# leducthanhig/image-restoration-models

Hardware: AMD Instinct MI355X
Metric: images/sec + PSNR, Restormer motion-deblur 1280x720 (higher is better)
Workload: dtype f32 (1x1 convs: fp32 emulated by 3 fp16 MFMAs on hi/lo operand splits with fp32 accumulation, error vs float64 at the level of an fp32 chain; everything else exact f32; value_exact_f32: f32 MFMA everywhere); 1 GPU; Restormer motion-deblur (WithBias LN, 26.13M params, synthetic weights seed 42) on 1280x720x3 uint8 GoPro-shaped synthetic frames; 6 tiles 512x512 (overlap 96) per frame; a step = 4 frame(s) per GPU, their 24 tiles in one batched forward; global_batch=4, tile=512, overlap=96, parallelism=per-image shard x1, no data-path collective

## Files before the change

image-restoration-models_amd/_hip.py:

```python
from __future__ import annotations

import ctypes as C
import os

import torch

_HERE = os.path.dirname(os.path.abspath(__file__))
LIB_PATH = os.path.join(_HERE, "libirm_hip.so")

ACT_NONE, ACT_RELU, ACT_GELU, ACT_SILU, ACT_RELU6 = 0, 1, 2, 3, 4
LN_NONE, LN_WITHBIAS, LN_BIASFREE = 0, 1, 2

_P, _L, _I, _F, _D = C.c_void_p, C.c_long, C.c_int, C.c_float, C.c_double

SIGNATURES = {
    "irm_version": [],
    "irm_ln_stats_f32": [_P, _L, _P, _I, _I, _I, _F, _P],
    "irm_gemm1x1_f32": [_P, _L, _P, _L, _P, _L, _P, _L, _P, _P, _P, _P, _I, _I, _I, _I, _I, _I, _I, _I, _P, _F, _P, _P],
    "irm_gemm1x1_f16x3_f32": [_P, _L, _P, _L, _P, _L, _P, _L, _P, _P, _P, _P, _I, _I, _I, _I, _I, _I, _I, _I, _P, _F, _P, _P],
    "irm_ln_split_f16": [_P, _L, _P, _P, _I, _F, _F, _P, _I, _I, _I, _P],
    "irm_ln_gemm_presplit_f16x3_f32": [_P, _P, _L, _P, _P, _I, _F, _F, _P, _L, _P, _F, _I, _I, _I, _I, _I, _P],
    "irm_ln_gemm_presplit_cl_f16x3_f32": [_P, _P, _L, _P, _P, _I, _F, _F, _P, _L, _P, _F, _I, _I, _I, _I, _I, _I, _P],
    "irm_gdfn_tail_f16x3_f32": [_P, _L, _P, _P, _P, _P, _L, _F, _I, _I, _I, _I, _I, _I, _P],
    "irm_gemm_presplit_f16x3_f32": [_P, _P, _P, _L, _P, _F, _I, _I, _I, _I, _I, _I, _I, _I, _P],
    "irm_dwconv3x3_f32": [_P, _L, _P, _P, _P, _L, _I, _I, _I, _I, _I, _P],
    "irm_dwconv3x3_gate_f32": [_P, _L, _P, _P, _P, _L, _I, _I, _I, _I, _P],
    "irm_dwgemm_f32": [_P, _L, _P, _P, _L, _P, _L, _P, _L, _P, _I, _I, _I, _I, _I, _I, _P, _F, _P],
    "irm_dwgemm_f16x3_f32": [_P, _L, _P, _P, _L, _P, _L, _P, _L, _P, _I, _I, _I, _I, _I, _I, _P, _F, _P],
    "irm_gdfn_fused_f16x3_f32": [_P, _P, _P, _P, _L, _P, _L, _I, _F, _F, _F, _I, _I, _I, _I, _I, _P],
    "irm_qkv_dw_fused_f16x3_f32": [_P, _P, _L, _P, _L, _I, _F, _F, _I, _I, _I, _I, _I, _P],
    "irm_mdta_gram_f32": [_P, _L, _P, _I, _I, _I, _I, _I, _P],
    "irm_mdta_gram_f16x3_f32": [_P, _L, _P, _P, _I, _I, _I, _I, _I, _P],
    "irm_mdta_finalize_f32": [_P, _P, _P, _P, _P, _P, _I, _I, _I, _I, _P],
    "irm_mdta_finalize_f16x3_f32": [_P, _P, _P, _P, _P, _P, _I, _I, _I, _I, _P],
    "irm_qkv_dw_fused_tm_f16x3_f32": [_P, _P, _L, _P, _L, _I, _F, _F, _I, _I, _I, _I, _I, _I, _P],
    "irm_qkv_gram_cm_f16x3_f32": [_P, _P, _L, _P, _L, _P, _P, _I, _F, _F, _I, _I, _I, _I, _I, _I, _P],
    "irm_qkv_dw_cm_f16x3_f32": [_P, _P, _L, _P, _L, _I, _F, _F, _I, _I, _I, _I, _I, _I, _P],
    "irm_mdta_gram_tm_f16x3_f32": [_P, _L, _P, _P, _I, _I, _I, _I, _I, _P],
    "irm_mdta_gram_tm_f32": [_P, _L, _P, _I, _I, _I, _I, _I, _P],
    "irm_mdta_finalize_frag_f16x3_f32": [_P, _P, _P, _P, _P, _P, _I, _I, _I, _I, _P],
    "irm_attn_gdfn_fused_f16x3_f32": [_P, _P, _P, _P, _L, _P, _L, _P, _P, _P, _L, _I, _F, _F, _F, _I, _I, _I, _I, _I, _I, _P],
    "irm_conv3x3_f32": [_P, _P, _L, _P, _L, _P, _L, _P, _I, _I, _I, _I, _I, _I, _I, _I, _I, _I, _I, _P],
    "irm_conv3x3_thin_f32": [_P, _P, _L, _P, _L, _P, _L, _P, _I, _I, _I, _I, _I, _I, _I, _I, _P],
    "irm_conv3x3_f16x3_f32": [_P, _F, _P, _L, _P, _L, _P, _L, _P, _I, _I, _I, _I, _I, _I, _I, _I, _I, _I, _I, _P],
    "irm_conv3x3_ep_f32": [_P, _P, _L, _P, _L, _P, _L, _P, _I, _I, _I, _I, _I, _I, _F, _I, _I, _I, _I, _I, _I, _P],
    "irm_conv3x3_f16x3_ep_f32": [_P, _F, _P, _L, _P, _L, _P, _L, _P, _I, _I, _I, _I, _I, _I, _F, _I, _I, _I, _I, _I, _I, _P],
    "irm_tile_extract": [_P, _I, _P, _P, _P, _I, _I, _I, _I, _I, _I, _I, _I, _F, _F, _I, _P],
    "irm_chan_stats_f32": [_P, _L, _P, _I, _I, _I, _F, _P],
    "irm_chan_stats_ws_f32": [_P, _L, _P, _P, _L, _I, _I, _I, _F, _P],
    "irm_chan_norm_act_f32": [_P, _L, _P, _P, _P, _P, _L, _P, _L, _I, _I, _I, _I, _P],
    "irm_conv3x3_s2_f32": [_P, _L, _P, _P, _L, _I, _I, _I, _I, _I, _P],
    "irm_dwconv3x3_s2_f32": [_P, _L, _P, _P, _L, _I, _I, _I, _I, _P],
    "irm_upsample_add_f32": [_P, _L, _P, _L, _P, _L, _I, _I, _I, _I, _I, _P],
    "irm_transpose_f32": [_P, _L, _P, _L, _I, _I, _I, _P],
    "irm_selective_scan_f32": [_P, _P, _P, _P, _P, _P, _P, _P, _P, _P, _P, _I, _I, _I, _I, _I, _I, _P],
    "irm_losh_combine_f32": [_P, _P, _P, _P, _P, _P, _P, _P, _L, _P, _L, _I, _I, _I, _I, _F, _P],
    "irm_window_blend": [_P, _P, _P, _P, _I, _P, _P, _I, _I, _I, _I, _I, _I, _I, _I, _I, _I, _F, _F, _P],
    "irm_window_blend_scaled": [_P, _P, _P, _P, _I, _P, _P, _I, _I, _I, _I, _I, _I, _I, _I, _I, _I, _I, _F, _F, _P],
    "irm_frame_metrics": [_P, _P, _I, _I, _I, _I, _I, _D, _P, _P, _P, _L, _P],
    "irm_imresize_bicubic": [_P, _I, _P, _I, _P, _P, _P, _P, _I, _I, _I, _I, _I, _I, _P],
    "irm_frame_metrics_basicsr": [_P, _P, _I, _I, _I, _I, _I, _I, _I, _I, _P, _P, _P, _L, _P],
    "irm_dihedral_chop_f32": [_P, _P, _P, _L, _I, _I, _I, _I, _I, _I, _I, _P],
    "irm_ensemble_merge_f32": [_P, _P, _P, _L, _I, _I, _I, _I, _I, _I, _P],
}

_lib = None


class HipLibraryError(RuntimeError):
    pass


def load():
    global _lib, LIB_PATH
    if _lib is None:
        if os.environ.get("IRM_HIP_LIB"):
            LIB_PATH = os.path.abspath(os.environ["IRM_HIP_LIB"])
        if not os.path.exists(LIB_PATH):
            raise HipLibraryError(
                f"{LIB_PATH} not found: build it with `python -c 'import __graft_entry__ as g; g.build()'` "
                "(make -C image-restoration-models_amd/csrc).  There is no CPU fallback.")
        lib = C.CDLL(LIB_PATH)
        for name, argtypes in SIGNATURES.items():
            fn = getattr(lib, name)
            fn.argtypes = argtypes
            fn.restype = _I
        _lib = lib
    return _lib


def _stream() -> int:
    return torch.cuda.current_stream().cuda_stream


def ptr(t):
    if t is None:
        return None
    if isinstance(t, int):
        return t
    assert t.is_cuda, "HIP kernels need device tensors"
    return t.data_ptr()


def call(name: str, *args):
    rc = getattr(load(), name)(*args, _stream())
    if rc != 0:
        raise HipLibraryError(f"{name} failed with status {rc} "
                              f"({'invalid arguments' if rc == -1 else 'HIP launch error'})")



def pack_gemm_weight(w: torch.Tensor) -> torch.Tensor:
    w = w.detach().reshape(w.shape[0], -1).float()
    m, k = w.shape
    mt, ks = (m + 15) // 16, 4 * ((k + 15) // 16)
    wpad = torch.zeros(mt * 16, ks * 4, dtype=torch.float32, device=w.device)
    wpad[:m, :k] = w
    return wpad.view(mt, 16, ks, 4).permute(0, 2, 3, 1).contiguous().view(-1)

# ... 381 lines not shown
```

image-restoration-models_amd/ops.py:

```python
from __future__ import annotations

import os

import torch

from . import _hip
from ._hip import ACT_GELU, ACT_NONE, ACT_RELU, ACT_RELU6, ACT_SILU, LN_BIASFREE, LN_NONE, LN_WITHBIAS


class KernelTimer:

    def __init__(self, detail=False, only=None):
        self.records = []
        self.detail = detail
        self.only = None if only is None else frozenset(only)
        self._chain = {}
        self._done = {}
        self._since = 0

    def _fold(self, k, e0, e1, fl, by):
        d = self._done.setdefault(k, dict(launches=0, ms=0.0, flops=0.0, bytes=0.0))
        d["launches"] += 1
        d["ms"] += e0.elapsed_time(e1)
        d["flops"] += fl
# ... 245 lines not shown
    ks = (C + 31) // 32
    return 2 * ks * ks * 512


def attn_gdfn_fused(pk, x, v, mfold_frag, y, C: int, hid: int, *, ln_mode, bias_o=None, bias=None, eps: float = 1e-5,
                    x_tm: bool = False, v_tm: bool = False, y_tm: bool = False):
    _chk(x, "x"), _chk(y, "y"), _chk(v, "v")
    B, _, H, W = x.shape
    assert x.data_ptr() != y.data_ptr() and x.shape[1] >= C and y.shape[1] >= C and v.shape[1] >= C and C % 16 == 0
    assert v.shape[0] == B and v.shape[2:] == x.shape[2:] and mfold_frag.numel() >= B * mfold_frag_numel(C)
    rec, w2, inv_s1, inv_s2 = pk
    N = H * W
    flops = B * N * (2.0 * C * C + 2.0 * 2 * hid * C + 36.0 * hid + 2.0 * hid * C)
    _launch("attn_gdfn_fused", flops, 4.0 * B * N * 3 * C, "irm_attn_gdfn_fused_f16x3_f32", _hip.ptr(rec), _hip.ptr(w2),
            _hip.ptr(bias), _hip.ptr(x), _bs(x), _hip.ptr(v), _bs(v), _hip.ptr(mfold_frag), _hip.ptr(bias_o),
            _hip.ptr(y), _bs(y), int(ln_mode), float(eps), float(inv_s1), float(inv_s2), B, C, hid, H, W,
            int(x_tm) | 2 * int(v_tm) | 4 * int(y_tm), tag=f"C{C} hid{hid} {H}x{W} B{B}")


def can_qk_tile_major(C: int, heads: int, H: int, W: int) -> bool:
    return C % 16 == 0 and C % heads == 0 and C // heads in (48, 96) and H % 8 == 0 and W % 32 == 0


def _use_qkv_cm(C: int) -> bool:
    return C <= 64


def qkv_dw_fused(pk, x, y, C: int, M: int, *, ln_mode, eps: float = 1e-5, tm: bool = False, x_tm: bool = False,
                 v_tm: bool = False):
    _chk(x, "x"), _chk(y, "y")
    B, _, H, W = x.shape
    assert x.data_ptr() != y.data_ptr() and x.shape[1] >= C and y.shape[1] >= M
    rec, inv_s1 = pk
    N = H * W
    if tm:
        assert M == 3 * C and y.shape[1] == M and H % 8 == 0 and W % 32 == 0
        _launch("qkv_dw_fused", B * N * (2.0 * M * C + 18.0 * M), 4.0 * B * N * (C + M),
                "irm_qkv_dw_cm_f16x3_f32" if _use_qkv_cm(C) else "irm_qkv_dw_fused_tm_f16x3_f32",
                _hip.ptr(rec), _hip.ptr(x), _bs(x), _hip.ptr(y), _bs(y), int(ln_mode), float(eps), float(inv_s1), B, C,
                H, W, int(x_tm), int(v_tm), tag=f"C{C} M{M} {H}x{W} B{B} tm")
        return
    assert not (x_tm or v_tm), "tile-major x / v need tm=True"
    _launch("qkv_dw_fused", B * N * (2.0 * M * C + 18.0 * M), 4.0 * B * N * (C + M), "irm_qkv_dw_fused_f16x3_f32",
            _hip.ptr(rec), _hip.ptr(x), _bs(x), _hip.ptr(y), _bs(y), int(ln_mode), float(eps), float(inv_s1), B, C, M,
            H, W, tag=f"C{C} M{M} {H}x{W} B{B}")


def mdta_plan(B: int, C: int, heads: int, N: int):
    c = C // heads
    sb = 3 if c % 48 == 0 else 2 if c % 32 == 0 else 1
    rec = c * c + 2 * c
    if c in (48, 96) and N % 64 == 0:
        slots, best = 2 * 256, None
        for chunk in range(128, 4096 + 1, 64):
            nchunk = -(-N // chunk)
            cost = -(-(B * heads * nchunk) // slots) * (chunk + 192)
            if best is None or cost < best[0]:
                best = (cost, chunk, nchunk)
        return best[1], best[2], rec
    nsub = (c // (16 * sb)) ** 2
    chunk = -(-(N * B * heads * nsub) // (4 * target_blocks()))
    chunk = min(max(-(-chunk // 64) * 64, 256), 4096)
    return chunk, -(-N // chunk), rec


QKV_GRAM_NCH = 4


def can_qkv_gram(C: int, heads: int, H: int, W: int) -> bool:
    return C == 48 and heads == 1 and H % 8 == 0 and W % 32 == 0 and ((H // 8) * (W // 32)) % QKV_GRAM_NCH == 0


def qkv_gram_cm(pk, x, y, gram_scale, part, C: int, *, ln_mode, eps: float = 1e-5, x_tm: bool = False, v_tm: bool = False) -> int:
    _chk(x, "x"), _chk(y, "y")
    B, _, H, W = x.shape
    assert can_qkv_gram(C, 1, H, W) and y.shape[1] == 3 * C and gram_scale.numel() == 2 * C
    rec, inv_s1 = pk
    N = H * W
    nchunk = (H // 8) * (W // 32) // QKV_GRAM_NCH
    assert part.numel() >= B * nchunk * (C * C + 2 * C)
    _launch("qkv_dw_fused", B * N * (2.0 * 3 * C * C + 18.0 * 3 * C + 2.0 * C * C), 4.0 * B * N * 2 * C, "irm_qkv_gram_cm_f16x3_f32",
            _hip.ptr(rec), _hip.ptr(x), _bs(x), _hip.ptr(y), _bs(y), _hip.ptr(gram_scale), _hip.ptr(part), int(ln_mode),
            float(eps), float(inv_s1), B, C, H, W, int(x_tm), int(v_tm), tag=f"C{C} {H}x{W} B{B} gram")
    return nchunk


def mdta_fold(qkv, part, gsum, temperature, wout, mfold, C: int, heads: int, attn=None, split: bool = False,
              gram_scale=None, frag: bool = False, tm: bool = False, nchunk_ready: int | None = None):
    _chk(qkv, "qkv")
    B, _, H, W = qkv.shape
    N = H * W
    chunk, nchunk, rec = mdta_plan(B, C, heads, N)
    if nchunk_ready is not None:
        nchunk = nchunk_ready
    assert part.numel() >= B * heads * nchunk * rec and gsum.numel() >= B * heads * rec
    c = C // heads
    assert not tm or (c in (48, 96) and N % 256 == 0), "tile-major q, k: the LDS-DMA ring passes only"
    if nchunk_ready is not None:
        pass
    elif gram_scale is not None and c in (48, 96) and N % 64 == 0:
        assert gram_scale.numel() == 2 * C and gram_scale.is_contiguous()
        _launch("mdta_gram_f16x3", 2.0 * B * heads * c * c * N, 8.0 * B * C * N,
                "irm_mdta_gram_tm_f16x3_f32" if tm else "irm_mdta_gram_f16x3_f32", _hip.ptr(qkv),
                _bs(qkv), _hip.ptr(gram_scale), _hip.ptr(part), B, C, heads, N, chunk,
                tag=f"C{C} h{heads} N{N} B{B} chunk{chunk}")
    else:
        _launch("mdta_gram", 2.0 * B * heads * c * c * N, 8.0 * B * C * N, "irm_mdta_gram_tm_f32" if tm else "irm_mdta_gram_f32",
                _hip.ptr(qkv), _bs(qkv), _hip.ptr(part), B, C, heads, N, chunk, tag=f"C{C} h{heads} N{N} B{B} chunk{chunk}")
    _launch("mdta_finalize", 2.0 * B * C * C * c, 4.0 * B * (heads * nchunk * rec + C * C),
            "irm_mdta_finalize_frag_f16x3_f32" if frag else "irm_mdta_finalize_f16x3_f32" if split else "irm_mdta_finalize_f32",
            _hip.ptr(part), _hip.ptr(gsum), _hip.ptr(temperature), _hip.ptr(wout), _hip.ptr(mfold), _hip.ptr(attn),
            B, C, heads, nchunk, tag=f"C{C} h{heads} nchunk{nchunk} B{B}")


def can_fuse_stats(M: int) -> bool:
    mt = (M + 15) // 16
    return mt <= _hip.choose_ct(mt)


def mfold_numel(C: int) -> int:
    mt = (C + 15) // 16
    return mt * 4 * mt * 64


def plan_conv3x3(co: int, H: int, W: int, B: int, *, split: bool, ct: int | None = None, ygroups: int | None = None):
    mt = (co + 15) // 16
    blocks = -(-W // 32) * -(-H // 8) * B
    if split:
        if ct is None:
            ct = 12 if mt >= 12 else 8 if mt >= 8 else 4 if mt % 4 == 0 else 3 if mt % 3 == 0 or mt > 4 else min(mt, 4)
            while ct > 1 and blocks * -(-mt // ct) < 256:
                ct = {12: 8, 8: 4}.get(ct, ct - 1)
        if ygroups is None:
            nchunks = -(-mt // ct)
            ygroups = max(1, min(nchunks, -(-512 // blocks)))
            while nchunks % ygroups:
                ygroups += 1
        return ct, ygroups
    if ct is None:
        ct = _hip.choose_ct(mt, (6, 4, 3, 2, 1))
        for smaller in (4, 3, 2, 1):
            if blocks * -(-mt // ct) >= 256 or smaller >= ct:
                continue
            ct = smaller
    if ygroups is None:
        nchunks = -(-mt // ct)
        ygroups = max(1, min(nchunks, -(-target_blocks() // blocks)))
    return ct, ygroups


def conv3x3(wp, x, y, ci: int, co: int, *, bias=None, relu1=False, res=None, res_mode=0, relu2=False,
            store_mode=0, ct: int | None = None, ygroups: int | None = None, leaky: float | None = None, shuffle: int = 2):
    _chk(x, "x"), _chk(y, "y")
    B, _, H, W = x.shape
    nbytes = 4.0 * B * H * W * (ci + co + (co if res is not None else 0))
    if leaky is not None and relu1:
        raise ValueError("conv3x3: relu1 and leaky are exclusive")
    act1, slope = (2, float(leaky)) if leaky is not None else (int(bool(relu1)), 0.0)
    extra = (f" ps{shuffle}" if shuffle != 2 else "") + (f" leaky{slope:g}" if leaky is not None else "")
    if isinstance(wp, _hip.ConvWeight):
        aligned = (W % 4 == 0 and _bs(x) % 4 == 0 and _bs(y) % 4 == 0 and _bs(res) % 4 == 0 and x.data_ptr() % 16 == 0
                   and y.data_ptr() % 16 == 0 and (res is None or res.data_ptr() % 16 == 0))
        if wp.raw is not None and aligned and store_mode == 0 and act1 < 2:
            _launch("conv3x3_thin", 18.0 * B * ci * co * H * W, nbytes, "irm_conv3x3_thin_f32", _hip.ptr(wp.raw), _hip.ptr(x),
                    _bs(x), _hip.ptr(y), _bs(y), _hip.ptr(res), _bs(res), _hip.ptr(bias), B, ci, co, H, W, int(relu1),
                    int(res_mode), int(relu2), tag=f"ci{ci} co{co} {H}x{W} B{B}")
# ... 96 lines not shown
```

image-restoration-models_amd/restormer/restormer.py:

```python
from __future__ import annotations

import os

import torch
import torch.nn as nn

from .. import _hip, ops

SYNTH_RULES = (
    (r"^output\.weight$", "gain", 0.02),
    (r"^skip_conv\.weight$", "gain", 0.5),
)


def _hidden(dim, factor):
    return int(dim * factor)


class _Norm(nn.Module):

    def __init__(self, dim, kind):
        super().__init__()
        self.body = nn.Module()
        self.body.weight = nn.Parameter(torch.ones(dim))
# ... 150 lines not shown
                    if gs is not None:
                        pk[name]["gram_s"] = gs.to(a.qkv.weight.device)
                if self._split and ops.can_fuse_gdfn(m.dim, 4):
                    pk[name].update(
                        qkv_f=_hip.pack_qkv_fused(a.qkv.weight, a.qkv.bias, a.qkv_dwconv.weight, a.qkv_dwconv.bias,
                                                  m.norm1.w, m.norm1.b),
                        gdfn_f=_hip.pack_gdfn_fused(ff.project_in.weight, ff.project_in.bias, ff.dwconv.weight,
                                                    ff.dwconv.bias, ff.project_out.weight, m.norm2.w, m.norm2.b))
                    if pk[name]["mfold_split"] and m.dim % 16 == 0:
                        pk[name]["gdfn_fa"] = _hip.pack_gdfn_fused(
                            ff.project_in.weight, ff.project_in.bias, ff.dwconv.weight, ff.dwconv.bias,
                            ff.project_out.weight, m.norm2.w, m.norm2.b, kperm=True)
                if ops.can_fuse_dw(m.dim, 4):
                    c, dw, dwb = m.dim, a.qkv_dwconv.weight.reshape(-1, 9), a.qkv_dwconv.bias
                    pk[name].update(
                        v_dwp=_hip.pack_dw_table(dw[2 * c:], None if dwb is None else dwb[2 * c:], c, False),
                        ffn_dwp=_hip.pack_dw_table(ff.dwconv.weight, ff.dwconv.bias, ff.hidden, True))
        for name in ("down1_2", "down2_3", "down3_4", "up4_3", "up3_2", "up2_1"):
            pk[name] = _hip.pack_conv3x3(getattr(self, name).body[0].weight)
        pk["patch_embed"] = _hip.pack_conv3x3(self.patch_embed.proj.weight)
        pk["patch_embed_b"] = f32(self.patch_embed.proj.bias)
        pk["output"] = _hip.pack_conv3x3(self.output.weight)
        pk["output_b"] = f32(self.output.bias)
        for name in ("reduce_chan_level3", "reduce_chan_level2") + (("skip_conv",) if self.dual_pixel_task else ()):
            pk[name] = _hip.pack_gemm_weight(getattr(self, name).weight)
            pk[name + "_b"] = f32(getattr(self, name).bias)
            if self._split and name != "skip_conv" and _hip.split_is_safe(getattr(self, name).weight):
                pk[name + "_s"] = _hip.pack_gemm_weight_split(getattr(self, name).weight)
        self._packed, self._packed_key = pk, key
        return pk

    @property
    def _ws(self):
        return self._ws_by_stream.setdefault(torch.cuda.current_stream().cuda_stream if torch.cuda.is_available()
                                             else 0, {})

    def _buf(self, name, numel, device):
        ws = self._ws
        t = ws.get(name)
        if t is None or t.numel() < numel or t.device != device:
            t = torch.empty(int(numel), dtype=torch.float32, device=device)
            ws[name] = t
        return t[:numel]

    def _zeros(self, key, numel, device):
        ws = self._ws
        t = ws.get(key)
        if t is None or t.device != device:
            t = torch.zeros(numel, dtype=torch.float32, device=device)
            ws[key] = t
        return t

    def release_workspace(self):
        self._ws_by_stream.clear()

    def _block(self, blk: TransformerBlock, w: dict, x: torch.Tensor, have_stats: bool = False,
               want_stats: bool = True) -> bool:
        B, C, H, W = x.shape
        N = H * W
        dev = x.device
        heads = blk.attn.num_heads
        hid = blk.ffn.hidden
        fuse = ops.can_fuse_stats(C)
        stats = self._buf("stats", B * 2 * N, dev)
        big_a = self._buf("scratch_a", B * max(3 * C, 2 * hid) * N, dev)
        big_b = self._buf("scratch_b", B * max(3 * C, hid) * N, dev)
        qkv = big_a[:B * 3 * C * N].view(B, 3 * C, H, W)
        qkv2 = big_b[:B * 3 * C * N].view(B, 3 * C, H, W)
        split = self._split and N % 4 == 0
        s_qkv, s_pin, s_pout = split and "qkv_s" in w, split and "pin_s" in w, split and "pout_s" in w
        s_fold = split and w.get("mfold_split", False)
        presplit = split and "qkv_ps" in w and ops.can_presplit(C, N)
        if presplit:
            xs = self._buf("xsplit", B * C * N, dev)
            frag, out_scale, s_x = w["qkv_ps"]
            ops.ln_gemm_presplit(frag, x, qkv, 3 * C, C, w["n1w"], w["n1b"], blk.norm1.mode, s_x, out_scale=out_scale,
                                 bias=w["qkv_b"], xs=xs)
        else:
            if not have_stats:
                ops.ln_stats(x, stats)
            ops.gemm1x1(w["qkv_s" if s_qkv else "qkv"], x, qkv, 3 * C, C, bias=w["qkv_b"], stats=stats, lnw=w["n1w"],
                        lnb=w["n1b"], ln_mode=blk.norm1.mode, split=s_qkv)
        fuse_dw = "v_dwp" in w and ops.can_fuse_dw(C, W)
        if fuse_dw:
            ops.dwconv3x3(qkv[:, :2 * C], w["qkv_dw"], qkv2[:, :2 * C],
                          bias=None if w["qkv_dw_b"] is None else w["qkv_dw_b"][:2 * C])
        else:
            ops.dwconv3x3(qkv, w["qkv_dw"], qkv2, bias=w["qkv_dw_b"])
        _, nchunk, rec = ops.mdta_plan(B, C, heads, N)
        part = self._buf("gram_part", B * heads * nchunk * rec, dev)
        gsum = self._buf("gram_sum", B * heads * rec, dev)
        mfold_n = ops.mfold_numel(C)
        mfold = self._zeros(("mfold", C, B), B * mfold_n, dev)
        ops.mdta_fold(qkv2, part, gsum, w["temp"], w["wout"], mfold, C, heads, split=s_fold,
                      gram_scale=w.get("gram_s") if split else None)
        if fuse_dw:
            ops.dwgemm(mfold, w["v_dwp"], qkv[:, 2 * C:], x, C, C, gate=False, res=x, bias=w["wout_b"],
                       w_bs=mfold_n, stats_out=stats if fuse else None, split=s_fold)
        else:
            ops.gemm1x1(mfold, qkv2[:, 2 * C:], x, C, C, res=x, bias=w["wout_b"], w_bs=mfold_n,
                        stats_out=stats if fuse else None, split=s_fold)
        if split and "tail" in w and ops.can_gdfn_tail(C, H, W):
            frag, out_scale, s_x, bp, hp = w["pin_cl"]
            h_cl = self._buf("h_cl", B * 2 * hp * N, dev)
            ops.ln_gemm_presplit_cl(frag, x, h_cl, 2 * hp, C, w["n2w"], w["n2b"], blk.norm2.mode, s_x, out_scale=out_scale, bias=bp)
            ops.gdfn_tail(w["tail"], h_cl, x, C, hid, hp, bias=w["pout_b"])
            return False
        h = big_a[:B * 2 * hid * N].view(B, 2 * hid, H, W)
        g = big_b[:B * hid * N].view(B, hid, H, W)
        if presplit:
            frag, out_scale, s_x = w["pin_ps"]
            ops.ln_gemm_presplit(frag, x, h, 2 * hid, C, w["n2w"], w["n2b"], blk.norm2.mode, s_x, out_scale=out_scale,
                                 bias=w["pin_b"], xs=xs)
        else:
            if not fuse:
                ops.ln_stats(x, stats)
            ops.gemm1x1(w["pin_s" if s_pin else "pin"], x, h, 2 * hid, C, bias=w["pin_b"], stats=stats, lnw=w["n2w"],
                        lnb=w["n2b"], ln_mode=blk.norm2.mode, split=s_pin)
        emit = fuse and want_stats
        if fuse_dw:
            ops.dwgemm(w["pout_s" if s_pout else "pout"], w["ffn_dwp"], h, x, C, hid, gate=True, res=x,
                       bias=w["pout_b"], stats_out=stats if emit else None, split=s_pout)
        else:
            ops.dwconv3x3_gate(h, w["ffn_dw"], g, bias=w["ffn_dw_b"])
            ops.gemm1x1(w["pout_s" if s_pout else "pout"], g, x, C, hid, res=x, bias=w["pout_b"],
                        stats_out=stats if emit else None, split=s_pout)
        return emit

    def _block_fused(self, blk: TransformerBlock, w: dict, x: torch.Tensor, alt: torch.Tensor, x_tm: bool = False,
                     y_tm: bool = False) -> torch.Tensor:
        B, C, H, W = x.shape
        N = H * W
        dev = x.device
        heads, hid = blk.attn.num_heads, blk.ffn.hidden
        qkv = self._buf("scratch_a", B * 3 * C * N, dev).view(B, 3 * C, H, W)
        tm = ops.can_qk_tile_major(C, heads, H, W)
        fa = "gdfn_fa" in w
        assert not (x_tm or y_tm) or (tm and fa), "tile-major x / y: only between the kernels that understand them"
        v_tm = tm and fa
        gram_in_qkv = tm and "gram_s" in w and ops.can_qkv_gram(C, heads, H, W)
        _, nchunk, rec = ops.mdta_plan(B, C, heads, N)
        nready = None
        if gram_in_qkv:
            nchunk = (H // 8) * (W // 32) // ops.QKV_GRAM_NCH
        part = self._buf("gram_part", B * heads * nchunk * rec, dev)
        if gram_in_qkv:
            nready = ops.qkv_gram_cm(w["qkv_f"], x, qkv, w["gram_s"], part, C, ln_mode=blk.norm1.mode, x_tm=x_tm, v_tm=v_tm)
        else:
            ops.qkv_dw_fused(w["qkv_f"], x, qkv, C, 3 * C, ln_mode=blk.norm1.mode, tm=tm, x_tm=x_tm, v_tm=v_tm)
        gsum = self._buf("gram_sum", B * heads * rec, dev)
        mfold_n = ops.mfold_numel(C)
        mfold = self._zeros(("mfold", C, B), B * mfold_n, dev)
        s_fold = w.get("mfold_split", False)
        if fa:
            mfrag = self._zeros(("mfold_frag", C, B), B * ops.mfold_frag_numel(C), dev)
            ops.mdta_fold(qkv, part, gsum, w["temp"], w["wout"], mfrag, C, heads, gram_scale=w.get("gram_s"), frag=True, tm=tm,
                          nchunk_ready=nready)
            ops.attn_gdfn_fused(w["gdfn_fa"], x, qkv[:, 2 * C:], mfrag, alt, C, hid, ln_mode=blk.norm2.mode,
                                bias_o=w["wout_b"], bias=w["pout_b"], x_tm=x_tm, v_tm=v_tm, y_tm=y_tm)
            return alt
        ops.mdta_fold(qkv, part, gsum, w["temp"], w["wout"], mfold, C, heads, split=s_fold, gram_scale=w.get("gram_s"), tm=tm,
                      nchunk_ready=nready)
        ops.gemm1x1(mfold, qkv[:, 2 * C:], x, C, C, res=x, bias=w["wout_b"], w_bs=mfold_n, split=s_fold)
        ops.gdfn_fused(w["gdfn_f"], x, alt, C, hid, ln_mode=blk.norm2.mode, bias=w["pout_b"])
        return alt

    def _run_stage(self, name, pk, x, have_stats=False):
        names = (name,) if isinstance(name, str) else tuple(name)
        blocks = [(f"{n}.{i}", blk) for n in names for i, blk in enumerate(getattr(self, n))]
        B, C, H, W = x.shape
        if (len(blocks) and all("gdfn_f" in pk[k] for k, _ in blocks) and ops.can_fuse_gdfn(C, W) and (H * W) % 4 == 0
                and len({blk.attn.num_heads for _, blk in blocks}) == 1):
            cur, alt = x, self._buf(f"alt_{C}", B * C * H * W, x.device).view(B, C, H, W)
            heads = blocks[0][1].attn.num_heads
            act_tm = all("gdfn_fa" in pk[k] for k, _ in blocks) and ops.can_qk_tile_major(C, heads, H, W)
            for i, (k, blk) in enumerate(blocks):
                out = self._block_fused(blk, pk[k], cur, alt, x_tm=act_tm and i > 0, y_tm=act_tm and i + 1 < len(blocks))
                cur, alt = out, cur
# ... 77 lines not shown
```

include/irm_hip.h:

```cpp
#ifndef IRM_HIP_H
#define IRM_HIP_H

#ifdef __cplusplus
extern "C" {
#endif

typedef struct ihipStream_t* irm_stream_t;

#define IRM_OK 0
#define IRM_EINVAL (-1)
#define IRM_ELAUNCH (-2)

#define IRM_ACT_NONE 0
#define IRM_ACT_RELU 1
#define IRM_ACT_GELU 2
#define IRM_ACT_SILU 3

#define IRM_LN_NONE 0
#define IRM_LN_WITHBIAS 1
#define IRM_LN_BIASFREE 2

int irm_version(void);

int irm_ln_stats_f32(const float* x, long x_bs, float* stats, int B, int C, int N, float eps,
                     irm_stream_t stream);

int irm_gemm1x1_f32(const float* wp, long w_bs, const float* x, long x_bs, float* y, long y_bs,
                    const float* res, long r_bs, const float* bias, const float* stats, const float* lnw,
                    const float* lnb, int ln_mode, int act, int B, int M, int K, int N, int ct, int ygroups,
                    float* stats_out, float eps, const float* res_scale, irm_stream_t stream);

int irm_gemm1x1_f16x3_f32(const float* wp_split, long w_bs, const float* x, long x_bs, float* y, long y_bs, const float* res,
                          long r_bs, const float* bias, const float* stats, const float* lnw, const float* lnb,
                          int ln_mode, int act, int B, int M, int K, int N, int ct, int ygroups, float* stats_out,
                          float eps, const float* res_scale, irm_stream_t stream);

int irm_ln_gemm_presplit_f16x3_f32(const void* wps, const float* x, long x_bs, const float* lnw, const float* lnb, int ln_mode,
                                   float x_scale, float eps, float* y, long y_bs, const float* bias, float out_scale, int B,
                                   int M, int K, int N, int mgroups, irm_stream_t stream);
int irm_ln_gemm_presplit_cl_f16x3_f32(const void* wps, const float* x, long x_bs, const float* lnw, const float* lnb, int ln_mode,
                                   float x_scale, float eps, float* y, long y_bs, const float* bias, float out_scale, int B,
                                   int M, int K, int H, int W, int mgroups, irm_stream_t stream);
int irm_ln_split_f16(const float* x, long x_bs, const float* lnw, const float* lnb, int ln_mode, float scale, float eps,
                     void* xs, int B, int K, int N, irm_stream_t stream);
int irm_gemm_presplit_f16x3_f32(const void* wps, const void* xs, float* y, long y_bs, const float* bias, float out_scale,
                                int act, int B, int M, int K, int N, int ct, int mgroups, int wg_shape,
                                irm_stream_t stream);

int irm_dwconv3x3_f32(const float* x, long x_bs, const float* w, const float* bias, float* y, long y_bs, int B,
                      int C, int H, int W, int act, irm_stream_t stream);

int irm_dwconv3x3_gate_f32(const float* x, long x_bs, const float* w, const float* bias, float* y, long y_bs,
                           int B, int hid, int H, int W, irm_stream_t stream);

int irm_dwgemm_f32(const float* wp, long w_bs, const float* dwp, const float* x, long x_bs, float* y, long y_bs,
                   const float* res, long r_bs, const float* bias, int gate, int B, int M, int K, int H, int W,
                   float* stats_out, float eps, irm_stream_t stream);

int irm_dwgemm_f16x3_f32(const float* wp_split, long w_bs, const float* dwp, const float* x, long x_bs, float* y, long y_bs,
                         const float* res, long r_bs, const float* bias, int gate, int B, int M, int K, int H, int W,
                         float* stats_out, float eps, irm_stream_t stream);

int irm_gdfn_fused_f16x3_f32(const float* rec, const float* w2, const float* bias2, const float* x, long x_bs, float* y,
                             long y_bs, int ln_mode, float eps, float inv_s1, float inv_s2, int B, int C, int hid, int H,
                             int W, irm_stream_t stream);
int irm_qkv_dw_fused_f16x3_f32(const float* rec, const float* x, long x_bs, float* y, long y_bs, int ln_mode, float eps,
                               float inv_s1, int B, int C, int M, int H, int W, irm_stream_t stream);
int irm_qkv_dw_fused_tm_f16x3_f32(const float* rec, const float* x, long x_bs, float* y, long y_bs, int ln_mode, float eps,
                                  float inv_s1, int B, int C, int H, int W, int x_tm, int v_tm, irm_stream_t stream);
int irm_qkv_dw_cm_f16x3_f32(const float* rec, const float* x, long x_bs, float* y, long y_bs, int ln_mode, float eps,
                            float inv_s1, int B, int C, int H, int W, int x_tm, int v_tm, irm_stream_t stream);
int irm_qkv_gram_cm_f16x3_f32(const float* rec, const float* x, long x_bs, float* y, long y_bs, const float* gscale, float* part,
                              int ln_mode, float eps, float inv_s1, int B, int C, int H, int W, int x_tm, int v_tm,
                              irm_stream_t stream);
int irm_attn_gdfn_fused_f16x3_f32(const float* rec, const float* w2, const float* bias2, const float* x, long x_bs,
                                  const float* v, long v_bs, const float* mfold_frag, const float* bias_o, float* y,
                                  long y_bs, int ln_mode, float eps, float inv_s1, float inv_s2, int B, int C, int hid,
                                  int H, int W, int lay, irm_stream_t stream);

int irm_gdfn_tail_f16x3_f32(const float* h_cl, long h_bs, const float* rec, const float* w2, const float* bias2, float* x,
                            long x_bs, float inv_s2, int B, int C, int hid, int hid_pad, int H, int W, irm_stream_t stream);

int irm_mdta_gram_f32(const float* qkv, long bs, float* part, int B, int C, int heads, int N, int chunk,
                      irm_stream_t stream);

int irm_mdta_gram_f16x3_f32(const float* qkv, long bs, const float* scale, float* part, int B, int C, int heads, int N,
                            int chunk, irm_stream_t stream);
int irm_mdta_gram_tm_f16x3_f32(const float* qkv, long bs, const float* scale, float* part, int B, int C, int heads, int N,
                            int chunk, irm_stream_t stream);
int irm_mdta_gram_tm_f32(const float* qkv, long bs, float* part, int B, int C, int heads, int N, int chunk,
                         irm_stream_t stream);

int irm_mdta_finalize_f32(const float* part, float* gsum, const float* temperature, const float* wout,
                          float* mfold, float* attn, int B, int C, int heads, int nchunk, irm_stream_t stream);
int irm_mdta_finalize_f16x3_f32(const float* part, float* gsum, const float* temperature, const float* wout,
                                float* mfold_split, float* attn, int B, int C, int heads, int nchunk,
                                irm_stream_t stream);
int irm_mdta_finalize_frag_f16x3_f32(const float* part, float* gsum, const float* temperature, const float* wout,
                                     float* mfold_frag, float* attn, int B, int C, int heads, int nchunk,
                                     irm_stream_t stream);

int irm_conv3x3_f32(const float* wp, const float* x, long x_bs, float* y, long y_bs, const float* res, long r_bs,
                    const float* bias, int B, int Ci, int Co, int H, int W, int relu1, int res_mode, int relu2,
                    int store_mode, int ct, int ygroups, irm_stream_t stream);

int irm_conv3x3_thin_f32(const float* w, const float* x, long x_bs, float* y, long y_bs, const float* res, long r_bs,
                         const float* bias, int B, int Ci, int Co, int H, int W, int relu1, int res_mode, int relu2,
                         irm_stream_t stream);

int irm_conv3x3_f16x3_f32(const float* wp_split, float inv_scale, const float* x, long x_bs, float* y, long y_bs,
                          const float* res, long r_bs, const float* bias, int B, int Ci, int Co, int H, int W, int relu1,
                          int res_mode, int relu2, int store_mode, int ct, int ygroups, irm_stream_t stream);

int irm_conv3x3_ep_f32(const float* wp, const float* x, long x_bs, float* y, long y_bs, const float* res, long r_bs,
                       const float* bias, int B, int Ci, int Co, int H, int W, int act1, float slope, int res_mode,
                       int relu2, int store_mode, int shuffle, int ct, int ygroups, irm_stream_t stream);
int irm_conv3x3_f16x3_ep_f32(const float* wp_split, float inv_scale, const float* x, long x_bs, float* y, long y_bs,
                             const float* res, long r_bs, const float* bias, int B, int Ci, int Co, int H, int W,
                             int act1, float slope, int res_mode, int relu2, int store_mode, int shuffle, int ct,
                             int ygroups, irm_stream_t stream);

int irm_tile_extract(const void* img, int is_u16, const int* origins, const double* noise, float* tiles, int H,
                     int W, int C, int th, int tw, int ph, int pw, int T, float mean, float inv_std, int pad_zero,
                     irm_stream_t stream);

int irm_window_blend(const float* pred, const int* origins, const float* window, void* out, int is_u16,
                     const void* target, unsigned long long* sse, int H, int W, int Co, int Cp, int th, int tw,
                     int ph, int pw, int ps, int T, float post_scale, float post_shift, irm_stream_t stream);

int irm_window_blend_scaled(const float* pred, const int* origins, const float* window, void* out, int is_u16,
                            const void* target, unsigned long long* sse, int H, int W, int Co, int Cp, int th, int tw,
                            int ph, int pw, int ps, int T, int scale, float post_scale, float post_shift,
                            irm_stream_t stream);

int irm_frame_metrics(const void* pred, const void* target, int is_u16, int K, int H, int W, int C, double data_range,
                      unsigned long long* sse, double* ssim, void* ws, long ws_words, irm_stream_t stream);

int irm_imresize_bicubic(const void* in, int is_u16, void* out, int out_float, const float* wh, const int* ih,
                         const float* ww, const int* iw, int K, int H, int W, int C, int s, int shrink,
                         irm_stream_t stream);

int irm_frame_metrics_basicsr(const void* pred, const void* target, int is_u16, int K, int H, int W, int C,
                              int crop_border, int test_y_channel, int bgr, void* sse, double* ssim, void* ws,
                              long ws_words, irm_stream_t stream);

int irm_chan_stats_f32(const float* x, long x_bs, float* stats, int B, int C, int N, float eps, irm_stream_t stream);
int irm_chan_stats_ws_f32(const float* x, long x_bs, float* stats, float* ws, long ws_floats, int B, int C, int N,
                          float eps, irm_stream_t stream);
int irm_chan_norm_act_f32(const float* x, long x_bs, const float* stats, const float* w, const float* b,
                          const float* res, long r_bs, float* y, long y_bs, int B, int C, int N, int act,
                          irm_stream_t stream);
int irm_conv3x3_s2_f32(const float* x, long x_bs, const float* w, float* y, long y_bs, int B, int Ci, int Co, int H,
                       int W, irm_stream_t stream);
int irm_dwconv3x3_s2_f32(const float* x, long x_bs, const float* w, float* y, long y_bs, int B, int C, int H, int W,
                         irm_stream_t stream);
int irm_upsample_add_f32(const float* src, long s_bs, const float* add, long a_bs, float* out, long o_bs, int B, int C,
                         int Hs, int Ws, int scale, irm_stream_t stream);
// ... 22 lines not shown
```

Before: 21.72 images/s.

## Fuse q/k depthwise conv with MDTA gram partials in one persistent kernel

Adds a persistent kernel for heads of width 48 (C=192/384) that applies the 3x3 depthwise conv to the q, k and v channels. It streams input tiles into LDS with a double-buffered global-to-LDS DMA ring. The q and k results feed the gram-matrix MFMA accumulation and norm sums directly and are never written to memory; only v is stored. This removes the write and re-read of the q/k planes between the dwconv and gram kernels, and the separate gram pass. mdta_fold is told the partial chunks are ready. The cost is a more complex kernel with large LDS use and a different chunking of gram partials.

```diff
diff --git a/image-restoration-models_amd/_hip.py b/image-restoration-models_amd/_hip.py
--- a/image-restoration-models_amd/_hip.py
+++ b/image-restoration-models_amd/_hip.py
@@ -35,6 +35,7 @@
     "irm_mdta_finalize_f16x3_f32": [_P, _P, _P, _P, _P, _P, _I, _I, _I, _I, _P],
     "irm_qkv_dw_fused_tm_f16x3_f32": [_P, _P, _L, _P, _L, _I, _F, _F, _I, _I, _I, _I, _I, _I, _P],
     "irm_qkv_gram_cm_f16x3_f32": [_P, _P, _L, _P, _L, _P, _P, _I, _F, _F, _I, _I, _I, _I, _I, _I, _P],
+    "irm_qkv_dw_gram_tail_f16x3_f32": [_P, _L, _P, _L, _P, _P, _P, _P, _I, _I, _I, _I, _I, _P],
     "irm_qkv_dw_cm_f16x3_f32": [_P, _P, _L, _P, _L, _I, _F, _F, _I, _I, _I, _I, _I, _I, _P],
     "irm_mdta_gram_tm_f16x3_f32": [_P, _L, _P, _P, _I, _I, _I, _I, _I, _P],
     "irm_mdta_gram_tm_f32": [_P, _L, _P, _I, _I, _I, _I, _I, _P],
diff --git a/image-restoration-models_amd/csrc/fused_qk_tail.hip b/image-restoration-models_amd/csrc/fused_qk_tail.hip
--- /dev/null
+++ b/image-restoration-models_amd/csrc/fused_qk_tail.hip
@@ -0,0 +1,302 @@
+#include "irm_common.h"
+#include <utility>
+
+typedef _Float16 qt_h8 __attribute__((ext_vector_type(8)));
+typedef float qt_v2 __attribute__((ext_vector_type(2)));
+
+#define QT_TH 8
+#define QT_TW 32
+#define QT_PITCH 36
+#define QT_SLOTS ((QT_TH + 2) * QT_PITCH)
+#define QT_CS 1728
+#define QT_IMG (32 * QT_CS)
+#define QT_NCH 4
+#define QT_REC (48 * 48 + 96)
+#define QT_TAP_B (5 * 10 * 32 * 4)
+#define QT_RED_OFF QT_TAP_B
+#define QT_PL_OFF (QT_RED_OFF + 4 * QT_REC * 4)
+#define QT_LDS (QT_PL_OFF + 2 * QT_IMG)
+static_assert(QT_PL_OFF % 16 == 0 && QT_LDS <= 160 * 1024, "LDS");
+static_assert(15 * 16 + QT_SLOTS * 4 <= QT_CS, "row + phase shift inside the row stride");
+
+__device__ __attribute__((aligned(16))) float qt_zero_page[4] = {0.f, 0.f, 0.f, 0.f};
+
+struct QtArgs {
+    const float* X; long x_bs;
+    float* V; long v_bs;
+    const float* taps;
+    const float* bias;
+    const float* gscale;
+    float* part;
+    int C, heads, H, W;
+    int tiles_x, tiles, items, gpx;
+};
+
+typedef __attribute__((address_space(3))) char qt_lc;
+__device__ __forceinline__ unsigned qt_opaque(unsigned v) { asm volatile("" : "+v"(v)); return v; }
+template <typename T>
+__device__ __forceinline__ T qt_ld(const qt_lc* base, unsigned voff, int imm) {
+    return *reinterpret_cast<const __attribute__((address_space(3))) T*>(base + voff + imm);
+}
+template <class F, int... Is>
+__device__ __forceinline__ void qt_for_impl(F&& f, std::integer_sequence<int, Is...>) { (f(std::integral_constant<int, Is>{}), ...); }
+template <int N, class F>
+__device__ __forceinline__ void qt_for(F&& f) { qt_for_impl(f, std::make_integer_sequence<int, N>{}); }
+__device__ __forceinline__ unsigned qt_row(int c) {
+    const int i = c & 15;
+    const int rk = i < 4 ? i : i < 12 ? i - 4 : i - 8;
+    const int o = (rk >> 1) * 4 + (rk & 1);
+    const int fix = (16 - ((c * (QT_CS / 16)) & 15)) & 15;
+    return (unsigned)(c * QT_CS + 16 * ((o + fix) & 15));
+}
+
+__global__ __launch_bounds__(512) void qk_tail_kernel(QtArgs a) {
+    IRM_KERNEL_ENTRY();
+    extern __shared__ __attribute__((aligned(16))) float smem[];
+    qt_lc* lds = (qt_lc*)smem;
+
+    const int wave = __builtin_amdgcn_readfirstlane((int)threadIdx.x >> 6);
+    const long plane = (long)a.H * a.W;
+    const int per = (a.items / QT_NCH + 7) >> 3;
+    const int xcd = blockIdx.x & 7, pos = blockIdx.x >> 3;
+    auto item_of = [&](int round) {
+        const int i = (round / QT_NCH) * a.gpx + pos;
+        return i < per ? (xcd * per + i) * QT_NCH + round % QT_NCH : a.items;
+    };
+
+    int round = 0;
+    int item = item_of(0);
+    if (item >= a.items) return;
+
+    int tid = threadIdx.x;
+    asm volatile("" : "+v"(tid));
+    const int lane = tid & 63, g = lane >> 4, r = lane & 15;
+    const unsigned vrow0 = qt_opaque(qt_row(r)), vrow1 = qt_opaque(qt_row(16 + r));
+
+    auto dma_stage = [&](int it, int st, int img) {
+        const int bh = it / a.tiles, tile = it - bh * a.tiles;
+        const int b = bh / a.heads, hd = bh - b * a.heads;
+        const int ty0 = (tile / a.tiles_x) * QT_TH, tx0 = (tile % a.tiles_x) * QT_TW;
+        const float* Xb = a.X + (long)b * a.x_bs;
+        int goff[6];
+#pragma unroll
+        for (int k = 0; k < 6; ++k) {
+            const int p = 64 * k + lane, ph = p / QT_PITCH, pc = p - ph * QT_PITCH;
+            const int gy = ty0 - 1 + ph, gx = tx0 - 1 + pc;
+            const bool inside = p < QT_SLOTS && pc < QT_TW + 2 && gy >= 0 && gy < a.H && gx >= 0 && gx < a.W;
+            goff[k] = inside ? gy * a.W + gx : -1;
+        }
+        const int nch = st < 4 ? 4 : 2;
+#pragma unroll
+        for (int ci = 0; ci < 4; ++ci) {
+            if (ci < nch) {
+                const int cl = nch * wave + ci;
+                const int j = 32 * st + cl;
+                const int pt = j / 48;
+                const float* src0 = Xb + (long)(pt * a.C + hd * 48 + (j - 48 * pt)) * plane;
+                float* dst = smem + (QT_PL_OFF + img * QT_IMG + (int)qt_row(cl)) / 4;
+#pragma unroll
+                for (int k = 0; k < 6; ++k) {
+                    const float* src = goff[k] >= 0 ? src0 + goff[k] : qt_zero_page;
+                    if (k < 5 || lane < QT_SLOTS - 320)
+                        __builtin_amdgcn_global_load_lds((const __attribute__((address_space(1))) void*)src,
+                                                         (__attribute__((address_space(3))) void*)(dst + 64 * k), 4, 0, 0);
+                }
+            }
+        }
+    };
+
+    f32x4 gacc[3][3];
+    float gnq[3] = {0.f, 0.f, 0.f}, gnk[3] = {0.f, 0.f, 0.f};
+#pragma unroll
+    for (int x = 0; x < 3; ++x)
+#pragma unroll
+        for (int y = 0; y < 3; ++y) gacc[x][y] = (f32x4){0.f, 0.f, 0.f, 0.f};
+    float gsc[6] = {1.f, 1.f, 1.f, 1.f, 1.f, 1.f};
+
+    dma_stage(item, 0, 0);
+    int cur = 0;
+    for (;;) {
+        const int bh = item / a.tiles, tile = item - bh * a.tiles;
+        const int b = bh / a.heads, hd = bh - b * a.heads;
+        const int ty0 = (tile / a.tiles_x) * QT_TH, tx0 = (tile % a.tiles_x) * QT_TW;
+        const int nitem = item_of(round + 1);
+
+        if (round % QT_NCH == 0) {
+            for (int e = threadIdx.x; e < 5 * 10 * 32; e += 512) {
+                const int st = e / 320, t = (e - st * 320) >> 5, j = 32 * st + (e & 31);
+                float val = 0.f;
+                if (j < 144) {
+                    const int pt = j / 48, gch = pt * a.C + hd * 48 + (j - 48 * pt);
+                    val = t < 9 ? a.taps[gch * 9 + t] : a.bias ? a.bias[gch] : 0.f;
+                }
+                smem[e] = val;
+            }
+#pragma unroll
+            for (int u = 0; u < 6; ++u) gsc[u] = a.gscale[(u / 3) * a.C + hd * 48 + 16 * (u % 3) + r];
+            asm volatile("s_waitcnt vmcnt(0) lgkmcnt(0)" ::: "memory");
+            __builtin_amdgcn_s_barrier();
+        }
+
+        f32x4 sp0[2][3], sp1[2][3];
+        qt_v2 sp2[2][3];
+        float stap[2][10];
+        auto st_read = [&](int st, int img, auto HC) {
+            constexpr int hct = decltype(HC)::value;
+            const unsigned vr = (hct ? vrow1 : vrow0) + (unsigned)((wave * QT_PITCH + 8 * g) * 4) + (unsigned)(img * QT_IMG);
+            const unsigned vt = (unsigned)((16 * hct + r) * 4);
+#pragma unroll
+            for (int dy = 0; dy < 3; ++dy) {
+                sp0[hct][dy] = qt_ld<f32x4>(lds, vr, QT_PL_OFF + dy * QT_PITCH * 4);
+                sp1[hct][dy] = qt_ld<f32x4>(lds, vr, QT_PL_OFF + dy * QT_PITCH * 4 + 16);
+                sp2[hct][dy] = qt_ld<qt_v2>(lds, vr, QT_PL_OFF + dy * QT_PITCH * 4 + 32);
+            }
+#pragma unroll
+            for (int t = 0; t < 10; ++t) stap[hct][t] = qt_ld<float>(lds, vt, st * 1280 + t * 128);
+        };
+        qt_h8 gqh[3], gql[3];
+        auto st_comp = [&](auto HC, auto UC) {
+            constexpr int hct = decltype(HC)::value;
+            constexpr int U = decltype(UC)::value;
+            float o[8];
+#pragma unroll
+            for (int e = 0; e < 8; ++e) o[e] = stap[hct][9];
+#pragma unroll
+            for (int dy = 0; dy < 3; ++dy) {
+                const float P[10] = {sp0[hct][dy][0], sp0[hct][dy][1], sp0[hct][dy][2], sp0[hct][dy][3], sp1[hct][dy][0],
+                                     sp1[hct][dy][1], sp1[hct][dy][2], sp1[hct][dy][3], sp2[hct][dy][0], sp2[hct][dy][1]};
+#pragma unroll
+                for (int dx = 0; dx < 3; ++dx) {
+                    const float t = stap[hct][dy * 3 + dx];
+#pragma unroll
+                    for (int e = 0; e < 8; ++e) o[e] = fmaf(t, P[e + dx], o[e]);
+                }
+            }
+            if constexpr (U < 6) {
+                const float sc = gsc[U];
+                float nn = 0.f, xs[8];
+#pragma unroll
+                for (int e = 0; e < 8; ++e) { nn = fmaf(o[e], o[e], nn); xs[e] = o[e] * sc; }
+                qt_h8 hi, lo;
+                irm_split8(xs, hi, lo);
+                if constexpr (U < 3) {
+                    gnq[U] += nn; gqh[U] = hi; gql[U] = lo;
+                } else {
+                    gnk[U - 3] += nn;
+#pragma unroll
+                    for (int x = 0; x < 3; ++x) {
+                        f32x4& t = gacc[x][U - 3];
+                        t = __builtin_amdgcn_mfma_f32_16x16x32_f16(gql[x], hi, t, 0, 0, 0);
+                        t = __builtin_amdgcn_mfma_f32_16x16x32_f16(gqh[x], lo, t, 0, 0, 0);
+                        t = __builtin_amdgcn_mfma_f32_16x16x32_f16(gqh[x], hi, t, 0, 0, 0);
+                    }
+                }
+            } else {
+                float* yt = a.V + (long)b * a.v_bs + (long)(hd * 48 + 16 * (U - 6) + r) * plane + (long)(ty0 + wave) * a.W + tx0 + 8 * g;
+                *reinterpret_cast<f32x4*>(yt) = (f32x4){o[0], o[1], o[2], o[3]};
+                *reinterpret_cast<f32x4*>(yt + 4) = (f32x4){o[4], o[5], o[6], o[7]};
+            }
+        };
+
+        constexpr std::integral_constant<int, 0> H0{};
+        constexpr std::integral_constant<int, 1> H1{};
+        qt_for<5>([&](auto STC) {
+            constexpr int st = decltype(STC)::value;
+            if constexpr (st < 4) dma_stage(item, st + 1, cur ^ 1);
+            else if (nitem < a.items) dma_stage(nitem, 0, cur ^ 1);
+            st_read(st, cur, H0);
+            if constexpr (st < 4) st_read(st, cur, H1);
+            st_comp(H0, std::integral_constant<int, 2 * st>{});
+            if constexpr (st < 4) st_comp(H1, std::integral_constant<int, 2 * st + 1>{});
+            asm volatile("s_waitcnt vmcnt(0) lgkmcnt(0)" ::: "memory");
+            __builtin_amdgcn_s_barrier();
+            cur ^= 1;
+        });
+
+        if (round % QT_NCH == QT_NCH - 1) {
+#pragma unroll
+            for (int t = 0; t < 3; ++t) {
+                gnq[t] += __shfl_xor(gnq[t], 16); gnq[t] += __shfl_xor(gnq[t], 32);
+                gnk[t] += __shfl_xor(gnk[t], 16); gnk[t] += __shfl_xor(gnk[t], 32);
+            }
+            float* red = smem + QT_RED_OFF / 4;
+            auto write_mine = [&]() {
+                float* mine = red + (wave & 3) * QT_REC;
+                float isk[3];
+#pragma unroll
+                for (int y = 0; y < 3; ++y) isk[y] = 1.0f / gsc[3 + y];
+#pragma unroll
+                for (int x = 0; x < 3; ++x) {
+                    const f32x4 sq4 = *reinterpret_cast<const f32x4*>(a.gscale + hd * 48 + 16 * x + 4 * g);
+#pragma unroll
+                    for (int e = 0; e < 4; ++e) {
+                        const float isq = 1.0f / sq4[e];
+#pragma unroll
+                        for (int y = 0; y < 3; ++y) mine[(16 * x + 4 * g + e) * 48 + 16 * y + r] = gacc[x][y][e] * (isq * isk[y]);
+                    }
+                    if (g == 0) { mine[48 * 48 + 16 * x + r] = gnq[x]; mine[48 * 48 + 48 + 16 * x + r] = gnk[x]; }
+                }
+            };
+            constexpr int NE = (QT_REC + 511) / 512;
+            float sum[NE];
+            if (wave < 4) write_mine();
+            __syncthreads();
+#pragma unroll
+            for (int i = 0; i < NE; ++i) {
+                const int e = threadIdx.x + 512 * i;
+                sum[i] = 0.f;
+                if (e < QT_REC) {
+                    sum[i] = red[e];
+#pragma unroll
+                    for (int w = 1; w < 4; ++w) sum[i] += red[w * QT_REC + e];
+                }
+            }
+            __syncthreads();
+            if (wave >= 4) write_mine();
+            __syncthreads();
+            float* out = a.part + ((long)bh * (a.tiles / QT_NCH) + tile / QT_NCH) * QT_REC;
+#pragma unroll
+            for (int i = 0; i < NE; ++i) {
+                const int e = threadIdx.x + 512 * i;
+                if (e < QT_REC) {
+#pragma unroll
+                    for (int w = 0; w < 4; ++w) sum[i] += red[w * QT_REC + e];
+                    out[e] = sum[i];
+                }
+            }
+#pragma unroll
+            for (int x = 0; x < 3; ++x) {
+                gnq[x] = 0.f; gnk[x] = 0.f;
+#pragma unroll
+                for (int y = 0; y < 3; ++y) gacc[x][y] = (f32x4){0.f, 0.f, 0.f, 0.f};
+            }
+        }
+        if (nitem >= a.items) break;
+        item = nitem;
+        ++round;
+    }
+}
+
+extern "C" int irm_qkv_dw_gram_tail_f16x3_f32(const float* qkv_pre, long bs, float* y_v, long y_bs, const float* taps,
+                                              const float* bias, const float* gscale, float* part, int B, int C, int heads, int H,
+                                              int W, hipStream_t stream) {
+    if (!qkv_pre || !y_v || !taps || !gscale || !part || qkv_pre == y_v || B <= 0 || heads <= 0 || H <= 0 || W <= 0) return IRM_EINVAL;
+    if ((C != 192 && C != 384) || C != 48 * heads || (H & 7) || (W & 31) || ((H / 8) * (W / 32)) % QT_NCH) return IRM_EINVAL;
+    if ((long)3 * C * H * W >= (1L << 30) || (long)B * heads * (H / 8) * (W / 32) >= (1L << 30)) return IRM_EINVAL;
+    if ((bs & 3) || (y_bs & 3) || !irm_aligned16(qkv_pre) || !irm_aligned16(y_v) || !irm_aligned16(gscale)) return IRM_EINVAL;
+    QtArgs a;
+    a.X = qkv_pre; a.x_bs = bs; a.V = y_v; a.v_bs = y_bs; a.taps = taps; a.bias = bias; a.gscale = gscale; a.part = part;
+    a.C = C; a.heads = heads; a.H = H; a.W = W;
+    a.tiles_x = W / QT_TW;
+    a.tiles = a.tiles_x * (H / QT_TH);
+    a.items = B * heads * a.tiles;
+    IRM_ALLOW_BIG_LDS((&qk_tail_kernel));
+    int dev = 0, n = 0;
+    if (hipGetDevice(&dev) != hipSuccess ||
+        hipDeviceGetAttribute(&n, hipDeviceAttributeMultiprocessorCount, dev) != hipSuccess || n <= 0) return IRM_ELAUNCH;
+    const int per = (a.items / QT_NCH + 7) >> 3;
+    a.gpx = (n + 7) / 8;
+    if (a.gpx > per) a.gpx = per;
+    hipLaunchKernelGGL(qk_tail_kernel, dim3(a.gpx * 8), dim3(512), QT_LDS, stream, a);
+    return irm_launch_status();
+}
diff --git a/image-restoration-models_amd/ops.py b/image-restoration-models_amd/ops.py
--- a/image-restoration-models_amd/ops.py
+++ b/image-restoration-models_amd/ops.py
@@ -351,6 +351,26 @@
     _launch("qkv_dw_fused", B * N * (2.0 * 3 * C * C + 18.0 * 3 * C + 2.0 * C * C), 4.0 * B * N * 2 * C, "irm_qkv_gram_cm_f16x3_f32",
             _hip.ptr(rec), _hip.ptr(x), _bs(x), _hip.ptr(y), _bs(y), _hip.ptr(gram_scale), _hip.ptr(part), int(ln_mode),
             float(eps), float(inv_s1), B, C, H, W, int(x_tm), int(v_tm), tag=f"C{C} {H}x{W} B{B} gram")
+    return nchunk
+
+
+def can_qk_tail(C: int, heads: int, H: int, W: int) -> bool:
+    return (C in (192, 384) and C == 48 * heads and H % 8 == 0 and W % 32 == 0
+            and ((H // 8) * (W // 32)) % QKV_GRAM_NCH == 0 and 3 * C * H * W < 1 << 30)
+
+
+def qk_tail(qkv_pre, v, w9, gram_scale, part, C: int, heads: int, *, bias=None) -> int:
+    _chk(qkv_pre, "qkv_pre"), _chk(v, "v")
+    B, _, H, W = qkv_pre.shape
+    assert can_qk_tail(C, heads, H, W) and qkv_pre.shape[1] == 3 * C and v.shape[1] >= C and v.shape[2:] == qkv_pre.shape[2:]
+    assert gram_scale.numel() == 2 * C and gram_scale.is_contiguous() and w9.numel() == 27 * C and w9.is_contiguous()
+    assert bias is None or (bias.numel() == 3 * C and bias.is_contiguous())
+    N = H * W
+    nchunk = (H // 8) * (W // 32) // QKV_GRAM_NCH
+    assert part.numel() >= B * heads * nchunk * (48 * 48 + 96)
+    _launch("qk_tail", B * N * (18.0 * 3 * C + 2.0 * 48 * C), 4.0 * B * N * 4 * C, "irm_qkv_dw_gram_tail_f16x3_f32",
+            _hip.ptr(qkv_pre), _bs(qkv_pre), _hip.ptr(v), _bs(v), _hip.ptr(w9), _hip.ptr(bias), _hip.ptr(gram_scale),
+            _hip.ptr(part), B, C, heads, H, W, tag=f"C{C} h{heads} {H}x{W} B{B}")
     return nchunk
 
 
diff --git a/image-restoration-models_amd/restormer/restormer.py b/image-restoration-models_amd/restormer/restormer.py
--- a/image-restoration-models_amd/restormer/restormer.py
+++ b/image-restoration-models_amd/restormer/restormer.py
@@ -256,18 +256,24 @@
             ops.gemm1x1(w["qkv_s" if s_qkv else "qkv"], x, qkv, 3 * C, C, bias=w["qkv_b"], stats=stats, lnw=w["n1w"],
                         lnb=w["n1b"], ln_mode=blk.norm1.mode, split=s_qkv)
         fuse_dw = "v_dwp" in w and ops.can_fuse_dw(C, W)
-        if fuse_dw:
+        qk_tail = split and not fuse_dw and "gram_s" in w and ops.can_qk_tail(C, heads, H, W)
+        _, nchunk, rec = ops.mdta_plan(B, C, heads, N)
+        if qk_tail:
+            nchunk = (H // 8) * (W // 32) // ops.QKV_GRAM_NCH
+        part = self._buf("gram_part", B * heads * nchunk * rec, dev)
+        nready = None
+        if qk_tail:
+            nready = ops.qk_tail(qkv, qkv2[:, 2 * C:], w["qkv_dw"], w["gram_s"], part, C, heads, bias=w["qkv_dw_b"])
+        elif fuse_dw:
             ops.dwconv3x3(qkv[:, :2 * C], w["qkv_dw"], qkv2[:, :2 * C],
                           bias=None if w["qkv_dw_b"] is None else w["qkv_dw_b"][:2 * C])
         else:
             ops.dwconv3x3(qkv, w["qkv_dw"], qkv2, bias=w["qkv_dw_b"])
-        _, nchunk, rec = ops.mdta_plan(B, C, heads, N)
-        part = self._buf("gram_part", B * heads * nchunk * rec, dev)
         gsum = self._buf("gram_sum", B * heads * rec, dev)
         mfold_n = ops.mfold_numel(C)
         mfold = self._zeros(("mfold", C, B), B * mfold_n, dev)
         ops.mdta_fold(qkv2, part, gsum, w["temp"], w["wout"], mfold, C, heads, split=s_fold,
-                      gram_scale=w.get("gram_s") if split else None)
+                      gram_scale=w.get("gram_s") if split else None, nchunk_ready=nready)
         if fuse_dw:
             ops.dwgemm(mfold, w["v_dwp"], qkv[:, 2 * C:], x, C, C, gate=False, res=x, bias=w["wout_b"],
                        w_bs=mfold_n, stats_out=stats if fuse else None, split=s_fold)
diff --git a/include/irm_hip.h b/include/irm_hip.h
--- a/include/irm_hip.h
+++ b/include/irm_hip.h
@@ -73,6 +73,9 @@
 int irm_qkv_gram_cm_f16x3_f32(const float* rec, const float* x, long x_bs, float* y, long y_bs, const float* gscale, float* part,
                               int ln_mode, float eps, float inv_s1, int B, int C, int H, int W, int x_tm, int v_tm,
                               irm_stream_t stream);
+int irm_qkv_dw_gram_tail_f16x3_f32(const float* qkv_pre, long bs, float* y_v, long y_bs, const float* taps, const float* bias,
+                                   const float* gscale, float* part, int B, int C, int heads, int H, int W,
+                                   irm_stream_t stream);
 int irm_attn_gdfn_fused_f16x3_f32(const float* rec, const float* w2, const float* bias2, const float* x, long x_bs,
                                   const float* v, long v_bs, const float* mfold_frag, const float* bias_o, float* y,
                                   long y_bs, int ln_mode, float eps, float inv_s1, float inv_s2, int B, int C, int hid,
```

Measured after the change: 21.80 images/s (median of 6 runs). Within noise of the previous version (+0.4%).
